# gorse-io/gorse

Measured on AMD Instinct MI355X. Metric: BPR positive-samples/sec (whole job, N GPUs), higher is better.
Workload: dtype f32; 1 GPU; S-ml1m 6040x3706x994169 per rank (C2), nFactors=64; factors_finite=True

## Files before the change

### gorse_amd/csrc/bpr.hip

```cpp
#include <algorithm>
#include <cstdlib>
#include <cstring>

#include "bpr_bins.hpp"
#include "mf_internal.hpp"
#include <utility>

using namespace gorse;

namespace {

int g_variant = 0;
constexpr int MODE_ATOMIC = GORSE_BPR_HOGWILD_ATOMIC;
constexpr int MODE_EXACT = GORSE_BPR_SEQUENTIAL;
constexpr int MODE_RACY = GORSE_BPR_HOGWILD_RACY;
constexpr int MODE_STORES = GORSE_BPR_HOGWILD_STORES;

__global__ __launch_bounds__(256) void bpr_sample_kernel(int32_t U, int32_t I, const int64_t *__restrict__ uptr,
                                                         const int32_t *__restrict__ uidx,
                                                         const int32_t *__restrict__ usorted, uint64_t seed,
                                                         uint64_t epoch, int64_t sample_base, int64_t n,
                                                         int32_t *__restrict__ us, int32_t *__restrict__ is,
                                                         int32_t *__restrict__ js, int32_t *__restrict__ fail_count) {
    for (int64_t s = (int64_t)blockIdx.x * blockDim.x + threadIdx.x; s < n; s += (int64_t)gridDim.x * blockDim.x) {
// ... 773 lines not shown
                for (int r = 0; r < RC; r++) v[b][r] = make_float2(0.0f, 0.0f);
                if (at[b] >= 0) {
                    const int32_t code = hot.meta[at[b] / d];
                    const int nr = 1 << hot_lg(code);
                    float *r0 = hot.rep + hot_base(code) * d + at[b] % d;
#pragma unroll
                    for (int r = 0; r < RC; r++)
                        if (rc + r < nr) v[b][r] = LAST ? drain_pair(r0 + (int64_t)(rc + r) * d) : load_pair(r0 + (int64_t)(rc + r) * d);
                }
            }
#pragma unroll
            for (int b = 0; b < BATCH; b++)
#pragma unroll
                for (int r = 0; r < RC; r++) sum[b].x += v[b][r].x, sum[b].y += v[b][r].y;
        }
#pragma unroll
        for (int b = 0; b < BATCH; b++)
            if (at[b] >= 0) {
                const float2 base = *(const float2 *)(hot.base + at[b]);
                store_pair(Q + (int64_t)hot.items[at[b] / d] * d + at[b] % d,
                           make_float2(sum[b].x != 0.0f ? base.x + sum[b].x : base.x, sum[b].y != 0.0f ? base.y + sum[b].y : base.y));
            }
    }
}

template <bool LAST>
__device__ void run_folders(const HotRows &hot, float *Q, int folders) {
    __shared__ int go;
    const int workers = (int)gridDim.x - folders;
    const int hotf = folders < kFolderBlocks ? folders : kFolderBlocks;
    const bool acc = (int)blockIdx.x >= hotf;
    const int n_all = hot.n_hot + hot.n_acc;
    const uint64_t period = acc ? (uint64_t)hot.period * (uint64_t)hot.acc_every : hot.period;
    if (blockIdx.x == 0 && threadIdx.x < kDoneStripes)
        __hip_atomic_store(done_set(hot, hot.set ^ 1) + threadIdx.x * kDoneStride, 0, __ATOMIC_RELAXED, __HIP_MEMORY_SCOPE_AGENT);
    bool sole = false;
    FoldShare sh{};
    if constexpr (LAST && GORSE_BPR_FOLD_SOLE_WRITER) {
        sole = hot.sole != 0;
        sh = fold_share((int)blockIdx.x, (int)threadIdx.x, hot.n_hot, hot.n_acc, folders, kFolderBlocks);
        if (sole) fold_sole_begin(hot, Q, sh);
    }
    const uint64_t t0 = wall_clock64();
    uint64_t next = t0 + period;
    int passes = 0;
    for (;;) {
        if (threadIdx.x < 64) {
            const bool all = workers_done(hot, workers);
            if (threadIdx.x == 0) {
                const uint64_t now = wall_clock64();
                int g = 0;
                if (all || now - t0 > hot.timeout) {
                    if constexpr (LAST) {
                        __builtin_amdgcn_fence(__ATOMIC_ACQUIRE, "agent");
                        asm volatile("s_waitcnt vmcnt(0)" ::: "memory");
                    }
                    g = 2;
                } else if (now >= next) {
                    next = now + period;
                    g = 1;
                }
                go = g;
            }
        }
        __syncthreads();
        const int g = go;
        __syncthreads();
        if (g == 0) continue;
        if (g == 2 && !LAST) break;
        const bool last = g == 2;
        if (sole) {
            if constexpr (LAST && GORSE_BPR_FOLD_SOLE_WRITER) {
                if (!acc) {
                    if (last)
                        fold_sole_pass<true, kHotReplicas, 1>(hot, Q, sh);
                    else
                        fold_sole_pass<false, kHotReplicas, 1>(hot, Q, sh);
                } else {
                    if (last)
                        fold_sole_pass<true, 1, 2>(hot, Q, sh);
                    else
                        fold_sole_pass<false, 1, 2>(hot, Q, sh);
                }
            }
        } else {
            const int first = last || !acc ? 0 : hotf, among = last ? folders : (acc ? folders - hotf : hotf);
            const int tid = ((int)blockIdx.x - first) * (int)blockDim.x + (int)threadIdx.x, nthreads = among * (int)blockDim.x;
            if (last || !acc) fold_pass(hot, Q, 0, hot.n_hot, tid, nthreads);
            if (last || acc) fold_acc_pass(hot, Q, hot.n_hot, n_all, tid, nthreads);
        }
        passes++;
        if (last) break;
    }
    if (threadIdx.x == 0 && ((int)blockIdx.x == 0 || (int)blockIdx.x == hotf)) hot.done[kFoldPassesWord + (acc ? 1 : 0)] = passes;
}

template <int NC, int MODE>
__global__ __launch_bounds__(kBlock) void bpr_update_kernel(float *P, float *Q, const int32_t *__restrict__ us,
                                                            const int32_t *__restrict__ is,
                                                            const int32_t *__restrict__ js,
                                                            const int32_t *__restrict__ order, int64_t begin,
                                                            int64_t end, int d, float lr, float reg, int exp_mode,
                                                            double *loss, HotRows hot, int folders) {
    extern __shared__ __attribute__((aligned(16))) float smem[];
    if (MODE == MODE_ATOMIC && (int)blockIdx.x < folders) {
        run_folders<false>(hot, Q, folders);
        return;
    }
    const int lane = threadIdx.x & (kGroup - 1);
    const int gib = threadIdx.x / kGroup;
    const int64_t group = (int64_t)((int)blockIdx.x - folders) * kGroupsPerBlock + gib;
    const int64_t ngroups = (int64_t)((int)gridDim.x - folders) * kGroupsPerBlock;
    const VecShape vs(d);
    const float nreg = -reg;
    double my_loss = 0.0;
    for (int64_t s = begin + group; s < end; s += ngroups) {
        const int64_t t = order ? (int64_t)order[s] : s;
        const int u = us[t], i = is[t], j = js[t];
        if ((u | i | j) < 0) continue;
        float *pu = P + (int64_t)u * d, *qi = Q + (int64_t)i * d, *qj = Q + (int64_t)j * d;
        float *qiw = qi;
        if (MODE == MODE_ATOMIC && folders > 0) {
            const int32_t code = hot.slot[i];
            if (code >= 0) qiw = hot_row(hot, code, group);
        }
        if constexpr (NC > 0) {
            float p[NC], a[NC], b[NC];
#pragma unroll
            for (int c = 0; c < NC; c++) {
                p[c] = load_row<MODE>(pu + 16 * c + lane);
                a[c] = load_row<MODE>(qi + 16 * c + lane);
                b[c] = load_row<MODE>(qj + 16 * c + lane);
            }
            const float diff = dot512_regs<NC>(p, a) - dot512_regs<NC>(p, b);
            const float ex = bpr_exp(-diff, exp_mode);
            const float grad = ex / (1.0f + ex);
            if (loss && lane == 0) my_loss += (double)log1pf(ex);
#pragma unroll
            for (int c = 0; c < NC; c++)
                update_elem<MODE>(pu, qiw, qj, 16 * c + lane, p[c], a[c], b[c], grad, nreg, lr, true, i == j);
        } else {
            float *sp = smem + (size_t)gib * 3 * d, *sa = sp + d, *sb = sa + d;
            for (int e = lane; e < d; e += kGroup) {
                sp[e] = load_row<MODE>(pu + e);
                sa[e] = load_row<MODE>(qi + e);
                sb[e] = load_row<MODE>(qj + e);
            }
            __builtin_amdgcn_wave_barrier();
            const float diff = dot512_lds(sp, sa, vs, lane) - dot512_lds(sp, sb, vs, lane);
            const float ex = bpr_exp(-diff, exp_mode);
            const float grad = ex / (1.0f + ex);
            if (loss && lane == 0) my_loss += (double)log1pf(ex);
            for (int e = lane; e < d; e += kGroup)
                update_elem<MODE>(pu, qiw, qj, e, sp[e], sa[e], sb[e], grad, nreg, lr, !vs.unfused(e), i == j);
            __builtin_amdgcn_wave_barrier();
        }
    }
    if (loss && lane == 0 && my_loss != 0.0) atomicAdd(loss, my_loss);
    if (MODE == MODE_ATOMIC && folders > 0) worker_done<false>(hot);
}

__global__ __launch_bounds__(256) void bpr_fold_kernel(HotRows hot, float *Q) {
    const int d = hot.d;
    const int64_t work = (int64_t)(hot.n_hot + hot.n_acc) * d;
    for (int64_t w = (int64_t)blockIdx.x * blockDim.x + threadIdx.x; w < work; w += (int64_t)gridDim.x * blockDim.x) {
        const int64_t slot = w / d;
        const int e = (int)(w - slot * d);
        const int32_t code = hot.meta[slot];
        float *r0 = hot.rep + hot_base(code) * d + e;
        float sum = 0.0f;
        for (int r = 0; r < (1 << hot_lg(code)); r++) {
            sum += r0[(int64_t)r * d];
            r0[(int64_t)r * d] = 0.0f;
        }
        if (sum != 0.0f) Q[(int64_t)hot.items[slot] * d + e] += sum;
    }
}

constexpr int kScanTile = 2048;

__global__ __launch_bounds__(256) void bpr_rank_kernel(const int32_t *__restrict__ key, int64_t n, int32_t K,
                                                       int32_t *__restrict__ bucket, int32_t *__restrict__ rank) {
    for (int64_t s = (int64_t)blockIdx.x * blockDim.x + threadIdx.x; s < n; s += (int64_t)gridDim.x * blockDim.x)
        rank[s] = atomicAdd(&bucket[key[s] < 0 ? K : key[s]], 1);
}

__device__ __forceinline__ int32_t block_exclusive_scan_256(int32_t v, int32_t *lds, int32_t *total) {
    const int lane = threadIdx.x & 63, wid = threadIdx.x >> 6;
    int32_t x = v;
#pragma unroll
    for (int o = 1; o < 64; o <<= 1) {
        int32_t y = __shfl_up(x, o, 64);
        if (lane >= o) x += y;
    }
    if (lane == 63) lds[wid] = x;
    __syncthreads();
    int32_t base = 0;
    for (int w = 0; w < wid; w++) base += lds[w];
    if (total) *total = lds[0] + lds[1] + lds[2] + lds[3];
    __syncthreads();
    return base + x - v;
}

__global__ __launch_bounds__(256) void scan_tile_sums_kernel(const int32_t *__restrict__ data, int64_t m,
                                                             int32_t *__restrict__ sums) {
    __shared__ int32_t lds[4];
    const int64_t base = (int64_t)blockIdx.x * kScanTile + (int64_t)threadIdx.x * 8;
    int32_t v = 0;
#pragma unroll
    for (int e = 0; e < 8; e++)
        if (base + e < m) v += data[base + e];
    int32_t total;
    (void)block_exclusive_scan_256(v, lds, &total);
    if (threadIdx.x == 0) sums[blockIdx.x] = total;
}

__global__ __launch_bounds__(256) void scan_sums_kernel(int32_t *__restrict__ sums, int64_t nt) {
    __shared__ int32_t lds[4];
    int32_t carry = 0;
    for (int64_t t0 = 0; t0 < nt; t0 += 256) {
        const int64_t t = t0 + threadIdx.x;
        const int32_t v = t < nt ? sums[t] : 0;
        int32_t total;
        const int32_t ex = block_exclusive_scan_256(v, lds, &total);
        if (t < nt) sums[t] = carry + ex;
        carry += total;
    }
}

__global__ __launch_bounds__(256) void scan_apply_kernel(int32_t *__restrict__ data, int64_t m,
                                                         const int32_t *__restrict__ sums) {
    __shared__ int32_t lds[4];
    const int64_t base = (int64_t)blockIdx.x * kScanTile + (int64_t)threadIdx.x * 8;
    int32_t x[8], v = 0;
#pragma unroll
    for (int e = 0; e < 8; e++) {
        x[e] = base + e < m ? data[base + e] : 0;
        v += x[e];
    }
    int32_t run = sums[blockIdx.x] + block_exclusive_scan_256(v, lds, nullptr);
#pragma unroll
    for (int e = 0; e < 8; e++) {
        if (base + e < m) data[base + e] = run;
        run += x[e];
    }
}


__global__ __launch_bounds__(256) void bpr_scatter_by_kernel(const int32_t *__restrict__ key, const int32_t *__restrict__ us,
                                                             const int32_t *__restrict__ is, const int32_t *__restrict__ js,
                                                             int64_t n, int32_t K, const int32_t *__restrict__ bucket,
                                                             const int32_t *__restrict__ rank, int32_t *__restrict__ su,
                                                             int32_t *__restrict__ si, int32_t *__restrict__ sj) {
    for (int64_t s = (int64_t)blockIdx.x * blockDim.x + threadIdx.x; s < n; s += (int64_t)gridDim.x * blockDim.x) {
        const int32_t kk = key[s] < 0 ? K : key[s];
        const int64_t pos = (int64_t)bucket[kk] + rank[s];
        su[pos] = us[s];
        si[pos] = is[s];
        sj[pos] = js[s];
    }
}

constexpr int kCold = -2;
constexpr int kSeriesFlush = 8;
#ifndef GORSE_BPR_SERIES_SKIP_GATHERS
#define GORSE_BPR_SERIES_SKIP_GATHERS 1
#endif

#ifndef GORSE_BPR_D8_PAIRS
#define GORSE_BPR_D8_PAIRS 1
#endif
template <int NC, bool NEG_STORE, bool D8 = false>
__global__ __launch_bounds__(kBlock) void bpr_update_user_kernel(float *P, float *Q, const int32_t *__restrict__ si,
                                                                 const int32_t *__restrict__ sj,
                                                                 const int32_t *__restrict__ off, int32_t U, int d,
                                                                 float lr, float reg, int exp_mode, double *loss,
                                                                 HotRows hot, int folders, int neg_replicas) {
    if ((int)blockIdx.x < folders) {
        run_folders<true>(hot, Q, folders);
        return;
    }
    auto continues = [](int i0, int j0, int i1, int j1) { return i0 == i1 && (i0 | j0 | j1) >= 0 && i0 != j0 && i0 != j1; };
    const int glane = threadIdx.x & (kGroup - 1);
    const int lane = D8 ? (glane & 7) : glane;
    constexpr int SUBS = D8 && GORSE_BPR_D8_PAIRS ? 2 : 1;
    const bool writer = !D8 || SUBS == 2 || glane < 8;
    auto mad = [](float x, float y, float z) { return D8 ? x * y + z : fmaf(x, y, z); };
    auto tree8 = [](float v) { return SUBS == 2 ? group_tree8_halves(v) : group_tree8(v); };
    const int gib = threadIdx.x / kGroup;
    const int64_t group = ((int64_t)((int)blockIdx.x - folders) * kGroupsPerBlock + gib) * SUBS + (SUBS == 2 ? glane >> 3 : 0);
    const int64_t ngroups = (int64_t)((int)gridDim.x - folders) * kGroupsPerBlock * SUBS;
    const float nreg = -reg;
    double my_loss = 0.0;
    const bool open = folders > 0;
    const bool look_i = open;
    const bool look_j = (open && neg_replicas) || NEG_STORE;
    const int32_t *slot_of = (look_i || look_j) ? hot.slot : si;
    int im1 = -1, jm1 = -1, im2 = -1, jm2 = -1;
    for (int64_t u = group; u < U; u += ngroups) {
        const int beg = off[u], end = off[u + 1];
        if (beg >= end) continue;
        float *pu = P + u * d;
        constexpr int G = 2, IA = 3;
        constexpr int GB = NEG_STORE ? 1 : G;
        float p[NC], ra[G][NC], rb[GB][NC];
        const int last = end - 1;
        auto at = [&](int s) { return s <= last ? s : last; };
        auto cl = [](int x) { return x < 0 ? 0 : x; };
        auto idx_i = [&](int i_, int j_) { return look_i ? cl(i_) : (look_j ? cl(j_) : beg); };
        auto idx_j = [&](int i_, int j_) { return look_j ? cl(j_) : (look_i ? cl(i_) : beg); };
        int ii[IA], jj[IA], sli[G], slj[G];
#pragma unroll
        for (int k = 0; k < IA; k++) ii[k] = si[at(beg + k)], jj[k] = sj[at(beg + k)];
#pragma unroll
        for (int k = 0; k < G; k++) sli[k] = slot_of[idx_i(ii[k], jj[k])], slj[k] = slot_of[idx_j(ii[k], jj[k])];
        float cur[NC], acc[NC];
        bool cont = false;
        int pending = 0;
#pragma unroll
        for (int c = 0; c < NC; c++) {
            p[c] = load_row<MODE_ATOMIC>(pu + 16 * c + lane);
#pragma unroll
            for (int k = 0; k < G; k++) ra[k][c] = load_row<MODE_ATOMIC>(Q + (int64_t)cl(ii[k]) * d + 16 * c + lane);
#pragma unroll
            for (int k = 0; k < GB; k++) rb[k][c] = load_row<MODE_ATOMIC>(Q + (int64_t)cl(jj[k]) * d + 16 * c + lane);
        }
        for (int s = beg; s < end; s++) {
            const int in_ = si[at(s + IA)], jn_ = sj[at(s + IA)];
            const int sli_n = slot_of[idx_i(ii[G], jj[G])];
            const int slj_n = slot_of[idx_j(ii[G], jj[G])];
            const int i = ii[0], j = jj[0], slot = sli[0], slotj = slj[0];
            float(&a)[NC] = ra[0];
            float(&b)[NC] = rb[0];
            float ran[NC], rbn[NC];
            const bool gather_i = !GORSE_BPR_SERIES_SKIP_GATHERS || !(s + G <= last && continues(ii[G - 1], jj[G - 1], ii[G], jj[G]));
#pragma unroll
            for (int c = 0; c < NC; c++) ran[c] = 0.0f;
            if (gather_i) {
#pragma unroll
                for (int c = 0; c < NC; c++) ran[c] = load_row<MODE_ATOMIC>(Q + (int64_t)cl(ii[G]) * d + 16 * c + lane);
            }
#pragma unroll
            for (int c = 0; c < NC; c++) rbn[c] = load_row<MODE_ATOMIC>(Q + (int64_t)cl(jj[GB]) * d + 16 * c + lane);
            if (cont) {
#pragma unroll
                for (int c = 0; c < NC; c++) a[c] = cur[c];
            }
            const bool more = s < last && continues(i, j, ii[1], jj[1]);
            const bool valid = j >= 0;
            float *qi = Q + (int64_t)cl(i) * d, *qj = Q + (int64_t)cl(j) * d;
            if (open && slot >= 0) qi = hot_row(hot, slot, group);
            if (open && neg_replicas && slotj >= 0) qj = hot_row(hot, slotj, group);
            bool st_j = false;
            if constexpr (NEG_STORE) {
                const bool own_j = i == j || j == im1 || j == jm1 || j == im2 || j == jm2;
                st_j = slotj == kCold && !own_j;
            }
            const float diff = D8 ? tree8(p[0] * a[0]) - tree8(p[0] * b[0]) : dot512_regs<NC>(p, a) - dot512_regs<NC>(p, b);
            const float ex = bpr_exp(-diff, exp_mode);
            const float grad = ex / (1.0f + ex);
            if (loss && (SUBS == 2 ? (glane & 7) == 0 : glane == 0) && valid) my_loss += (double)log1pf(ex);
            float t1[NC], t2[NC];
#pragma unroll
            for (int c = 0; c < NC; c++) {
                t1[c] = mad(a[c], nreg, p[c] * grad);
                t2[c] = mad(b[c], nreg, p[c] * (-grad));
                const float t3 = mad(p[c], nreg, (a[c] - b[c]) * grad);
                p[c] = valid ? mad(t3, lr, p[c]) : p[c];
            }
            if (valid) {
#pragma unroll
                for (int c = 0; c < NC; c++) {
                    acc[c] = pending > 0 ? acc[c] + t1[c] * lr : t1[c] * lr;
                    cur[c] = mad(t1[c], lr, a[c]);
                }
                if (!more || ++pending >= kSeriesFlush) {
                    pending = 0;
                    if (writer) {
#pragma unroll
                        for (int c = 0; c < NC; c++)
                            __hip_atomic_fetch_add(qi + 16 * c + lane, acc[c], __ATOMIC_RELAXED, __HIP_MEMORY_SCOPE_AGENT);
                    }
                }
            }
            cont = more;
            if (!valid || !writer) {
            } else if (st_j) {
#pragma unroll
                for (int c = 0; c < NC; c++)
                    __hip_atomic_store(qj + 16 * c + lane, mad(t2[c], lr, b[c]), __ATOMIC_RELAXED, __HIP_MEMORY_SCOPE_AGENT);
            } else {
#pragma unroll
                for (int c = 0; c < NC; c++)
                    __hip_atomic_fetch_add(qj + 16 * c + lane, t2[c] * lr, __ATOMIC_RELAXED, __HIP_MEMORY_SCOPE_AGENT);
            }
#pragma unroll
            for (int c = 0; c < NC; c++) {
#pragma unroll
                for (int k = 0; k + 1 < G; k++) ra[k][c] = ra[k + 1][c];
                ra[G - 1][c] = ran[c];
#pragma unroll
                for (int k = 0; k + 1 < GB; k++) rb[k][c] = rb[k + 1][c];
                rb[GB - 1][c] = rbn[c];
            }
            im2 = im1, jm2 = jm1, im1 = i, jm1 = j;
#pragma unroll
            for (int k = 0; k + 1 < IA; k++) ii[k] = ii[k + 1], jj[k] = jj[k + 1];
            ii[IA - 1] = in_, jj[IA - 1] = jn_;
#pragma unroll
            for (int k = 0; k + 1 < G; k++) sli[k] = sli[k + 1], slj[k] = slj[k + 1];
            sli[G - 1] = sli_n, slj[G - 1] = slj_n;
        }
        if (writer) {
#pragma unroll
            for (int c = 0; c < NC; c++)
                __hip_atomic_store(pu + 16 * c + lane, p[c], __ATOMIC_RELAXED, __HIP_MEMORY_SCOPE_AGENT);
        }
    }
    if (loss && (SUBS == 2 ? (glane & 7) == 0 : glane == 0) && my_loss != 0.0) atomicAdd(loss, my_loss);
    if (folders > 0) worker_done<true>(hot);
}

__global__ __launch_bounds__(256) void scan_small_kernel(int32_t *__restrict__ data, int64_t m) {
    __shared__ int32_t lds[4];
    int32_t carry = 0;
    for (int64_t t0 = 0; t0 < m; t0 += kScanTile) {
        const int64_t base = t0 + (int64_t)threadIdx.x * 8;
        int32_t x[8], v = 0;
#pragma unroll
        for (int e = 0; e < 8; e++) {
            x[e] = base + e < m ? data[base + e] : 0;
            v += x[e];
        }
        int32_t total;
        int32_t run = carry + block_exclusive_scan_256(v, lds, &total);
#pragma unroll
        for (int e = 0; e < 8; e++) {
            if (base + e < m) data[base + e] = run;
            run += x[e];
        }
        carry += total;
    }
}

int32_t exclusive_scan_i32(int32_t *data, int64_t m, int32_t *tmp, hipStream_t st) {
    const int64_t nt = ceil_div(m, kScanTile);
    if (nt <= 16) {
        scan_small_kernel<<<dim3(1), dim3(256), 0, st>>>(data, m);
        GORSE_HIP_CHECK(hipGetLastError());
        return GORSE_OK;
    }
    scan_tile_sums_kernel<<<dim3((unsigned)nt), dim3(256), 0, st>>>(data, m, tmp);
    scan_sums_kernel<<<dim3(1), dim3(256), 0, st>>>(tmp, nt);
    scan_apply_kernel<<<dim3((unsigned)nt), dim3(256), 0, st>>>(data, m, tmp);
    GORSE_HIP_CHECK(hipGetLastError());
    return GORSE_OK;
}


int32_t launch_user_sort(gorse_mf *h, const int32_t *trip, int32_t *sorted, int32_t *bucket, int32_t *rank, int64_t n, size_t cap,
                         hipStream_t st) {
    const int64_t m = h->U + 2;
    const int64_t blocks = std::min<int64_t>(ceil_div(n, 256), 256 * 8);
    GORSE_HIP_CHECK(hipMemsetAsync(bucket, 0, (size_t)m * sizeof(int32_t), st));
    if (g_variant & GORSE_TEST_BPR_STABLE_RANK)
        bpr_rank_kernel<<<dim3(1), dim3(1), 0, st>>>(trip, n, (int32_t)h->U, bucket, rank);
    else
        bpr_rank_kernel<<<dim3((unsigned)blocks), dim3(256), 0, st>>>(trip, n, (int32_t)h->U, bucket, rank);
    GORSE_TRY(exclusive_scan_i32(bucket, m, h->scan_tmp2.p, st));
    bpr_scatter_by_kernel<<<dim3((unsigned)blocks), dim3(256), 0, st>>>(trip, trip, trip + cap, trip + 2 * cap, n,
                                                                       (int32_t)h->U, bucket, rank, sorted,
                                                                       sorted + cap, sorted + 2 * cap);
    GORSE_HIP_CHECK(hipGetLastError());
    return GORSE_OK;
}
int32_t ensure_user_sort(gorse_mf *h) {
    const int64_t m = h->U + 2;
    const size_t mat = prep_matrix_words(h->U, (int64_t)h->trip_cap);
    if ((size_t)m <= h->ubucket[0].n && h->scan_tmp2.n >= (size_t)ceil_div(m, kScanTile) && h->urank[0].n >= 2 * h->trip_cap &&
        h->ubins.n >= (size_t)2 * kMaxBins && h->ubinmat.n >= mat)
        return GORSE_OK;
    GORSE_TRY(mf_sync_streams(h));
    if (h->ubins.n < (size_t)2 * kMaxBins) GORSE_TRY(h->ubins.alloc((size_t)2 * kMaxBins));
    if (h->ubinmat.n < mat) GORSE_TRY(h->ubinmat.alloc(mat));
    for (int b = 0; b < 2; b++) {
        GORSE_TRY(h->ubucket[b].alloc((size_t)m));
        GORSE_TRY(h->urank[b].alloc(2 * h->trip_cap));
    }
    if (h->scan_tmp2.n < (size_t)ceil_div(m, kScanTile)) GORSE_TRY(h->scan_tmp2.alloc((size_t)ceil_div(m, kScanTile)));
    return GORSE_OK;
}
bool user_runs_supported(const gorse_mf *h) {
    return (h->d == 8 || h->d == 16 || h->d == 32 || h->d == 64 || h->d == 128) && (h->U >= 4096 || (g_variant & GORSE_TEST_BPR_USER_RUNS));
}

constexpr int kDefaultStoreMode = 1;
int g_store_mode = kDefaultStoreMode;

HotRows make_hot(const gorse_mf *h) {
    return HotRows{h->hot_slot.p, h->hot_items.p, h->hot_meta.p, h->hot_rep.p, h->hot_done.p, 0, h->d, 0, g_fold_period, 0, g_acc_fold_every,
                   h->hot_base.p, 0, g_folder_timeout};
}
bool has_hot(const gorse_mf *h) { return h->n_hot > 0 || h->n_acc > 0; }
int open_hot(gorse_mf *h, HotRows &hot) {
    hot.n_hot = h->n_hot;
    hot.n_acc = h->n_acc;
    hot.set = (int)(h->hot_launches++ & 1);
    return kFolderBlocks + (h->n_acc > 0 ? kFolderBlocksAcc : 0);
}

int32_t launch_update_users(gorse_mf *h, const int32_t *sorted, const int32_t *bucket, size_t cap, float lr, float reg,
                            int exp_mode, double *loss, hipStream_t st, bool stores, hipEvent_t start = nullptr,
                            hipEvent_t stop = nullptr) {
    const int d = h->d;
    int64_t blocks = ceil_div(h->U, (int64_t)kGroupsPerBlock * (d == 8 && GORSE_BPR_D8_PAIRS ? 2 : 1));
    const int64_t capb = 256 * 16;
    if (blocks > capb) blocks = capb;
    HotRows hot = make_hot(h);
    const int folders = has_hot(h) ? open_hot(h, hot) : 0;
    blocks += folders;
    const int neg_rep = hot.n_acc > 0 || (hot.n_hot > 0 && hot_neg_replicas(hot.n_hot, h->I)) ? 1 : 0;
    dim3 grid((unsigned)blocks), block(kBlock);
    const bool neg_store = stores && h->n_cold > 0 && g_store_mode == 1;
    hot.sole = GORSE_BPR_FOLD_SOLE_WRITER && hot.n_acc > 0 && !neg_store && h->hot_base.p != nullptr ? 1 : 0;
    if (folders > 0) h->fold_sole_last = hot.sole;
#define LAUNCH2(NC, NEG_STORE)                                                                                         \
    hipExtLaunchKernelGGL((bpr_update_user_kernel<(NC == 0 ? 1 : NC), NEG_STORE, NC == 0>), grid, block, 0, st, start, stop, 0,     \
                          h->P.p, h->Q.p, sorted + cap, sorted + 2 * cap, bucket, (int32_t)h->U, d, lr, reg, exp_mode, loss, hot, \
                          folders, neg_rep)
#define LAUNCH(NC)                                                                                                     \
    do {                                                                                                               \
        if (neg_store)                                                                                                 \
            LAUNCH2(NC, true);                                                                                         \
        else                                                                                                           \
            LAUNCH2(NC, false);                                                                                        \
    } while (0)
    if (d == 8)
        LAUNCH(0);
    else if (d == 16)
        LAUNCH(1);
    else if (d == 32)
        LAUNCH(2);
    else if (d == 64)
        LAUNCH(4);
    else
        LAUNCH(8);
#undef LAUNCH2
#undef LAUNCH
    GORSE_HIP_CHECK(hipGetLastError());
    return GORSE_OK;
}

template <int MODE>
int32_t launch_update_mode(gorse_mf *h, const int32_t *us, const int32_t *is, const int32_t *js, const int32_t *order,
                           int64_t begin, int64_t end, float lr, float reg, int exp_mode, double *loss,
                           hipStream_t st, hipEvent_t start, hipEvent_t stop) {
    const int64_t n = end - begin;
    if (n <= 0) return GORSE_OK;
    const int d = h->d;
    int64_t blocks = ceil_div(n, kGroupsPerBlock);
    const int64_t cap = 256 * 16;
    if (blocks > cap) blocks = cap;
    HotRows hot = make_hot(h);
    const int folders = MODE == MODE_ATOMIC && has_hot(h) ? open_hot(h, hot) : 0;
    if (folders > 0) h->fold_sole_last = 0;
    blocks += folders;
    dim3 grid((unsigned)blocks), block(kBlock);
#define LAUNCH(NC, SH)                                                                                              \
    hipExtLaunchKernelGGL((bpr_update_kernel<NC, MODE>), grid, block, SH, st, start, folders > 0 ? nullptr : stop, 0, h->P.p, \
                          h->Q.p, us, is, js, order, begin, end, d, lr, reg, exp_mode, loss, hot, folders)
    if (d == 16)
        LAUNCH(1, 0);
    else if (d == 32)
        LAUNCH(2, 0);
    else if (d == 64)
        LAUNCH(4, 0);
    else if (d == 128)
        LAUNCH(8, 0);
    else
        LAUNCH(0, (size_t)kGroupsPerBlock * 3 * d * sizeof(float));
#undef LAUNCH
    GORSE_HIP_CHECK(hipGetLastError());
    if (folders > 0) {
        const int64_t fb = std::min<int64_t>(ceil_div((int64_t)(hot.n_hot + hot.n_acc) * d, 256), 512);
        hipExtLaunchKernelGGL(bpr_fold_kernel, dim3((unsigned)fb), dim3(256), 0, st, nullptr, stop, 0, hot, h->Q.p);
        GORSE_HIP_CHECK(hipGetLastError());
    }
    return GORSE_OK;
}

int32_t launch_update(gorse_mf *h, int mode, const int32_t *us, const int32_t *is, const int32_t *js,
                      const int32_t *order, int64_t begin, int64_t end, float lr, float reg, int exp_mode, double *loss,
                      hipStream_t st, hipEvent_t start = nullptr, hipEvent_t stop = nullptr) {
    switch (mode) {
    case MODE_ATOMIC:
        return launch_update_mode<MODE_ATOMIC>(h, us, is, js, order, begin, end, lr, reg, exp_mode, loss, st, start, stop);
    case MODE_EXACT:
        return launch_update_mode<MODE_EXACT>(h, us, is, js, order, begin, end, lr, reg, exp_mode, loss, st, start, stop);
    case MODE_RACY:
        return launch_update_mode<MODE_RACY>(h, us, is, js, order, begin, end, lr, reg, exp_mode, loss, st, start, stop);
    }
    return fail(GORSE_ERR_INVALID, "unknown BPR mode %d", mode);
}

int32_t launch_sampler(gorse_mf *h, uint64_t seed, uint64_t epoch, int64_t base, int64_t n, int32_t *trip, size_t cap,
                       hipStream_t st, hipEvent_t start = nullptr, hipEvent_t stop = nullptr) {
    if (n <= 0) return GORSE_OK;
    int64_t blocks = std::min<int64_t>(ceil_div(n, 256), 256 * 8);
    hipExtLaunchKernelGGL(bpr_sample_kernel, dim3((unsigned)blocks), dim3(256), 0, st, start, stop, 0, (int32_t)h->U, (int32_t)h->I,
                          h->uptr.p, h->uidx.p, h->uidx_sorted.p, seed, epoch, base, n, trip, trip + cap, trip + 2 * cap,
                          h->fail_count.p);
    GORSE_HIP_CHECK(hipGetLastError());
    return GORSE_OK;
}

constexpr size_t kItemsBatchFrom = (size_t)8 << 20;
int32_t launch_prepare_users(gorse_mf *h, uint64_t seed, uint64_t epoch, int64_t base, int64_t n, int32_t *trip, int32_t *sorted,
                             int32_t *bucket, int32_t *rank, size_t cap, hipStream_t st) {
    if (n <= 0) return GORSE_OK;
    const int64_t m = h->U + 2;
    const int64_t blocks = std::min<int64_t>(ceil_div(n, 256), 256 * 8);
    const PrepBins pb = prep_bins(h->U, n);
    hipEvent_t ev_a = nullptr, ev_b = nullptr;
    auto launch_items = [&](const int2 *pairs) {
        h->prof.events(GORSE_PROF_BPR_SAMPLE, &ev_a, &ev_b);
        if (h->uidx.n > kItemsBatchFrom)
            hipExtLaunchKernelGGL(bpr_sample_items_batch_kernel, dim3((unsigned)blocks), dim3(256), 0, st, ev_a, ev_b, 0, (int32_t)h->U,
                                  (int32_t)h->I, h->uptr.p, h->uidx.p, h->uidx_sorted.p, seed, epoch, base, n, pairs, sorted + cap,
                                  sorted + 2 * cap, h->fail_count.p);
        else
            hipExtLaunchKernelGGL(bpr_sample_items_kernel, dim3((unsigned)blocks), dim3(256), 0, st, ev_a, ev_b, 0, (int32_t)h->U,
                                  (int32_t)h->I, h->uptr.p, h->uidx.p, h->uidx_sorted.p, seed, epoch, base, n, pairs, sorted + cap,
                                  sorted + 2 * cap, h->fail_count.p);
    };
    auto launch_group = [&]() {
        if (g_variant & GORSE_TEST_BPR_ARRIVAL_ORDER) return;
        h->prof.events(GORSE_PROF_BPR_SORT, &ev_a, &ev_b);
        hipExtLaunchKernelGGL(bpr_group_positives_kernel, dim3((unsigned)std::min<int64_t>(h->U, 256 * 16)), dim3(64), 0, st, ev_a, ev_b, 0,
                              (int32_t)h->U, bucket, sorted + cap, sorted + 2 * cap);
    };
    if (pb.ok && !(g_variant & GORSE_TEST_BPR_NO_BINS)) {
        int32_t *key = trip;
        int2 *bp = reinterpret_cast<int2 *>(trip + cap), *pairs = reinterpret_cast<int2 *>(rank);
        int32_t *bin_count = h->ubins.p, *bin_start = h->ubins.p + kMaxBins, *H = h->ubinmat.p;
        const unsigned tiles = (unsigned)ceil_div(n, pb.tile);
        if ((size_t)tiles * pb.nbins > h->ubinmat.n) return fail(GORSE_ERR_INVALID, "tile x bin matrix smaller than %u x %d", tiles, pb.nbins);
        const bool finish = !(g_variant & GORSE_TEST_BPR_THREE_KERNELS) && pb.shift <= kFinShift && n / pb.nbins <= kFinCap / 4 * 3 &&
                            h->uidx.n <= kItemsBatchFrom;
        h->prof.events(GORSE_PROF_BPR_SAMPLE, &ev_a, &ev_b);
        hipExtLaunchKernelGGL(bpr_bin_count_kernel, dim3(tiles), dim3(kBinThreads), 0, st, ev_a, ev_b, 0, (int32_t)h->U, h->uptr.p, seed,
                              epoch, base, n, pb.tile, pb.shift, pb.nbins, key, h->fail_count.p, H);
        h->prof.events(GORSE_PROF_BPR_SORT, &ev_a, &ev_b);
        hipExtLaunchKernelGGL(bpr_bin_offsets_kernel, dim3((unsigned)ceil_div(pb.nbins, 64)), dim3(kOffWaves * 64), 0, st, ev_a, nullptr, 0,
                              H, (int)tiles, pb.nbins, bin_count);
        hipExtLaunchKernelGGL(bpr_bin_scatter_kernel, dim3(tiles), dim3(kBinThreads), 0, st, nullptr, finish ? ev_b : nullptr, 0,
                              (int32_t)h->U, key, n, pb.tile, pb.shift, pb.nbins, bin_count, H, bin_start, bp);
        if (finish) {
            h->prof.events(GORSE_PROF_BPR_SAMPLE, &ev_a, &ev_b);
            hipExtLaunchKernelGGL(bpr_bin_finish_kernel, dim3((unsigned)pb.nbins), dim3(kFinThreads), 0, st, ev_a, ev_b, 0, (int32_t)h->U,
                                  (int32_t)h->I, pb.shift, bin_start, bp, h->uptr.p, h->uidx.p, h->uidx_sorted.p, seed, epoch, base, bucket,
                                  pairs, sorted + cap, sorted + 2 * cap, h->fail_count.p, (g_variant & GORSE_TEST_BPR_ARRIVAL_ORDER) ? 0 : 1);
            GORSE_HIP_CHECK(hipGetLastError());
            return GORSE_OK;
        }
        hipExtLaunchKernelGGL(bpr_bin_sort_kernel, dim3((unsigned)pb.nbins), dim3(256), 0, st, nullptr, ev_b, 0, (int32_t)h->U, pb.shift,
                              pb.nbins, bin_start, bp, bucket, pairs);
        launch_items(pairs);
        launch_group();
        GORSE_HIP_CHECK(hipGetLastError());
        return GORSE_OK;
    }
    int32_t *key = trip;
    int2 *pairs = reinterpret_cast<int2 *>(trip + cap);
    int tok = h->prof.begin(GORSE_PROF_BPR_SAMPLE, st);
    GORSE_HIP_CHECK(hipMemsetAsync(bucket, 0, (size_t)m * sizeof(int32_t), st));
    bpr_sample_user_kernel<<<dim3((unsigned)blocks), dim3(256), 0, st>>>((int32_t)h->U, h->uptr.p, seed, epoch, base, n, key,
                                                                         h->fail_count.p, bucket, rank);
    h->prof.end(tok, st);
    tok = h->prof.begin(GORSE_PROF_BPR_SORT, st);
    GORSE_TRY(exclusive_scan_i32(bucket, m, h->scan_tmp2.p, st));
    bpr_scatter_ids_kernel<<<dim3((unsigned)blocks), dim3(256), 0, st>>>(key, rank, bucket, n, (int32_t)h->U, pairs);
    h->prof.end(tok, st);
    launch_items(pairs);
    launch_group();
    GORSE_HIP_CHECK(hipGetLastError());
    return GORSE_OK;
}

int64_t g_chunk_override = 0;
int64_t chunk_capacity(const gorse_mf *h) {
    if (g_chunk_override > 0) return g_chunk_override;
    const int64_t lo = (int64_t)1 << 22, hi = (int64_t)1 << 27;
    return std::min(std::max(lo, 32 * h->U), hi);
}

int32_t ensure_trip(gorse_mf *h, int64_t want) {
    size_t cap = (size_t)std::min<int64_t>(std::max<int64_t>(want, 1), chunk_capacity(h));
    cap = (cap + 1) & ~(size_t)1;
    if (cap <= h->trip_cap) return GORSE_OK;
    GORSE_TRY(mf_sync_streams(h));
    for (int b = 0; b < 2; b++) GORSE_TRY(h->trip[b].alloc(cap * 3));
    for (int b = 0; b < 2; b++) GORSE_TRY(h->sorted[b].alloc(cap * 3));
    h->trip_cap = cap;
    return GORSE_OK;
}

void build_levels(int64_t U, int64_t I, const int32_t *u, const int32_t *i, const int32_t *j, int64_t n,
                  std::vector<int32_t> &order, std::vector<int64_t> &level_ptr) {
    std::vector<int32_t> lastP((size_t)U, 0), lastQ((size_t)I, 0), lvl((size_t)n, 0);
    int32_t maxl = 0;
    for (int64_t s = 0; s < n; s++) {
        if ((u[s] | i[s] | j[s]) < 0) continue;
        int32_t l = std::max(lastP[u[s]], std::max(lastQ[i[s]], lastQ[j[s]])) + 1;
        lvl[s] = l;
// ... 317 lines not shown
```

Baseline: 2.599 billion samples/s.

## Replace shifting prefetch registers with a 4-slot ring unrolled by phase

The per-sample software pipeline used to shift the prefetched Q rows and index/slot arrays down by one slot every iteration. It now keeps them in a power-of-two ring indexed by the unrolled phase, which removes the register move chains. When rows are wide enough, the loop also leaves the unrolled block early through a wave ballot once no lane is still live. It adds an explicit waitcnt before the loop, and the larger ring arrays raise register pressure, which could lower occupancy or cause spills. Samples past the end of a row are masked as not live.

```diff
diff --git a/gorse_amd/csrc/bpr.hip b/gorse_amd/csrc/bpr.hip
--- a/gorse_amd/csrc/bpr.hip
+++ b/gorse_amd/csrc/bpr.hip
@@ -1099,14 +1099,17 @@
         if (beg >= end) continue;
         float *pu = P + u * d;
         constexpr int G = 2, IA = 3;
+        constexpr int R = 4;
+        static_assert(R > IA && IA > G && (R & (R - 1)) == 0, "a ring holds the current sample and the IA ahead of it");
         constexpr int GB = NEG_STORE ? 1 : G;
-        float p[NC], ra[G][NC], rb[GB][NC];
+        constexpr bool kLeaveTurn = NC >= 4 && !NEG_STORE;
+        float p[NC], ra[R][NC], rb[R][NC];
         const int last = end - 1;
         auto at = [&](int s) { return s <= last ? s : last; };
         auto cl = [](int x) { return x < 0 ? 0 : x; };
         auto idx_i = [&](int i_, int j_) { return look_i ? cl(i_) : (look_j ? cl(j_) : beg); };
         auto idx_j = [&](int i_, int j_) { return look_j ? cl(j_) : (look_i ? cl(i_) : beg); };
-        int ii[IA], jj[IA], sli[G], slj[G];
+        int ii[R], jj[R], sli[R], slj[R];
 #pragma unroll
         for (int k = 0; k < IA; k++) ii[k] = si[at(beg + k)], jj[k] = sj[at(beg + k)];
 #pragma unroll
@@ -1120,31 +1123,37 @@
 #pragma unroll
             for (int k = 0; k < G; k++) ra[k][c] = load_row<MODE_ATOMIC>(Q + (int64_t)cl(ii[k]) * d + 16 * c + lane);
 #pragma unroll
+            for (int k = G; k < R; k++) ra[k][c] = 0.0f;
+#pragma unroll
             for (int k = 0; k < GB; k++) rb[k][c] = load_row<MODE_ATOMIC>(Q + (int64_t)cl(jj[k]) * d + 16 * c + lane);
         }
-        for (int s = beg; s < end; s++) {
-            const int in_ = si[at(s + IA)], jn_ = sj[at(s + IA)];
-            const int sli_n = slot_of[idx_i(ii[G], jj[G])];
-            const int slj_n = slot_of[idx_j(ii[G], jj[G])];
-            const int i = ii[0], j = jj[0], slot = sli[0], slotj = slj[0];
-            float(&a)[NC] = ra[0];
-            float(&b)[NC] = rb[0];
-            float ran[NC], rbn[NC];
-            const bool gather_i = !GORSE_BPR_SERIES_SKIP_GATHERS || !(s + G <= last && continues(ii[G - 1], jj[G - 1], ii[G], jj[G]));
-#pragma unroll
-            for (int c = 0; c < NC; c++) ran[c] = 0.0f;
+        __builtin_amdgcn_s_waitcnt(0x0F70);
+        for (int s0 = beg; s0 < end; s0 += R) {
+#pragma unroll
+          for (int ph = 0; ph < R; ph++) {
+            constexpr int M = R - 1;
+            const int s = s0 + ph;
+            const bool live = s < end;
+            if (kLeaveTurn && ph > 0 && __builtin_amdgcn_ballot_w64(live) == 0) break;
+            const int n1 = (ph + 1) & M, nG = (ph + G) & M, nB = (ph + GB) & M, nA = (ph + IA) & M;
+            const int i = ii[ph], j = jj[ph];
+            ii[nA] = si[at(s + IA)], jj[nA] = sj[at(s + IA)];
+            sli[nG] = slot_of[idx_i(ii[nG], jj[nG])];
+            slj[nG] = slot_of[idx_j(ii[nG], jj[nG])];
+#pragma unroll
+            for (int c = 0; c < NC; c++) rb[nB][c] = load_row<MODE_ATOMIC>(Q + (int64_t)cl(jj[nB]) * d + 16 * c + lane);
+            const bool gather_i = !GORSE_BPR_SERIES_SKIP_GATHERS || !(s + G <= last && continues(ii[n1], jj[n1], ii[nG], jj[nG]));
             if (gather_i) {
 #pragma unroll
-                for (int c = 0; c < NC; c++) ran[c] = load_row<MODE_ATOMIC>(Q + (int64_t)cl(ii[G]) * d + 16 * c + lane);
-            }
-#pragma unroll
-            for (int c = 0; c < NC; c++) rbn[c] = load_row<MODE_ATOMIC>(Q + (int64_t)cl(jj[GB]) * d + 16 * c + lane);
-            if (cont) {
-#pragma unroll
-                for (int c = 0; c < NC; c++) a[c] = cur[c];
-            }
-            const bool more = s < last && continues(i, j, ii[1], jj[1]);
-            const bool valid = j >= 0;
+                for (int c = 0; c < NC; c++) ra[nG][c] = load_row<MODE_ATOMIC>(Q + (int64_t)cl(ii[nG]) * d + 16 * c + lane);
+            }
+            const int slot = sli[ph], slotj = slj[ph];
+            float a[NC];
+            const float(&b)[NC] = rb[ph];
+#pragma unroll
+            for (int c = 0; c < NC; c++) a[c] = cont ? cur[c] : ra[ph][c];
+            const bool more = s < last && continues(i, j, ii[n1], jj[n1]);
+            const bool valid = live && j >= 0;
             float *qi = Q + (int64_t)cl(i) * d, *qj = Q + (int64_t)cl(j) * d;
             if (open && slot >= 0) qi = hot_row(hot, slot, group);
             if (open && neg_replicas && slotj >= 0) qj = hot_row(hot, slotj, group);
@@ -1191,22 +1200,8 @@
                 for (int c = 0; c < NC; c++)
                     __hip_atomic_fetch_add(qj + 16 * c + lane, t2[c] * lr, __ATOMIC_RELAXED, __HIP_MEMORY_SCOPE_AGENT);
             }
-#pragma unroll
-            for (int c = 0; c < NC; c++) {
-#pragma unroll
-                for (int k = 0; k + 1 < G; k++) ra[k][c] = ra[k + 1][c];
-                ra[G - 1][c] = ran[c];
-#pragma unroll
-                for (int k = 0; k + 1 < GB; k++) rb[k][c] = rb[k + 1][c];
-                rb[GB - 1][c] = rbn[c];
-            }
-            im2 = im1, jm2 = jm1, im1 = i, jm1 = j;
-#pragma unroll
-            for (int k = 0; k + 1 < IA; k++) ii[k] = ii[k + 1], jj[k] = jj[k + 1];
-            ii[IA - 1] = in_, jj[IA - 1] = jn_;
-#pragma unroll
-            for (int k = 0; k + 1 < G; k++) sli[k] = sli[k + 1], slj[k] = slj[k + 1];
-            sli[G - 1] = sli_n, slj[G - 1] = slj_n;
+            if (NEG_STORE && live) im2 = im1, jm2 = jm1, im1 = i, jm1 = j;
+          }
         }
         if (writer) {
 #pragma unroll
```

Result: no change. 2.617 billion samples/s (median of 6 runs) (+0.7%).
